# Aqasch/TensorRL-QAS

Hardware: AMD Instinct MI355X
Metric: VQE env-steps/sec (higher is better)
Workload: dtype f64

## Files before the change

### include/vqe_hip.h

```cpp
#ifndef VQE_HIP_H
#define VQE_HIP_H

#include <stdint.h>

#ifdef __cplusplus
extern "C" {
#endif

typedef struct vqe_handle vqe_t;
typedef struct vqe_cobyla vqe_cobyla_t;

enum {
  VQE_OK = 0,
  VQE_EINVAL = -22,
  VQE_ENOMEM = -12,
  VQE_ENODEV = -19,
  VQE_EHIP = -5,
  VQE_ESTATE = -1
};

enum {
  VQE_GATE_CNOT = 0,
  VQE_GATE_RX = 1,
  VQE_GATE_RY = 2,
  VQE_GATE_RZ = 3,
  VQE_GATE_DEPOL1 = 4,
  VQE_GATE_DEPOL2 = 5
};

int vqe_create(int n_qubits, int device_id, vqe_t** out);
void vqe_destroy(vqe_t* h);
const char* vqe_last_error(const vqe_t* h);
int vqe_set_stream(vqe_t* h, void* hip_stream);
int vqe_get_stream(vqe_t* h, void** hip_stream);
int vqe_sync(vqe_t* h);
int vqe_device_info(vqe_t* h, int64_t info[4]);

int vqe_set_init_state(vqe_t* h, const double* amps_re_im );
int vqe_set_init_state_dev(vqe_t* h, const void* dev_amps_re_im);
int vqe_get_state_dev(vqe_t* h, const double* theta, void* dev_amps_re_im);
int vqe_set_hamiltonian_pauli(vqe_t* h, int n_terms, const uint64_t* xmask,
                              const uint64_t* zmask, const double* coeff);
int vqe_set_hamiltonian_dense(vqe_t* h, const double* op_re_im , double tol);
int vqe_hamiltonian_terms(vqe_t* h, int32_t* n_terms, int32_t* n_xgroups);
int vqe_hamiltonian_layout(vqe_t* h, int32_t out[4]);
int vqe_set_term_shard(vqe_t* h, int rank, int world);
int vqe_set_amplitude_shard(vqe_t* h, int rank, int world);
int vqe_comm_unique_id(void* id128);
int vqe_comm_init(vqe_t* h, int rank, int world, const void* id128);
int vqe_comm_allreduce_energy(vqe_t* h);
int vqe_comm_destroy(vqe_t* h);
int vqe_term_owner(int n_qubits, int n_terms, const uint64_t* xmask, int world, int32_t* owner);
int vqe_set_noise(vqe_t* h, double p1, double p2, uint64_t seed);
int vqe_set_noise_mode(vqe_t* h, int mode);
int vqe_dm_plan(int n_qubits, int n_gates, const int32_t* kind, const int32_t* q0, const int32_t* q1, const int32_t* param_idx,
                const double* theta, double p1, double p2, int cap_blocks, int32_t* n_blocks, int32_t* windows, double* S);
int vqe_noise_mode_info(vqe_t* h, int32_t out[2]);
int vqe_set_shot_noise(vqe_t* h, double sigma_total, uint64_t seed);

int vqe_set_circuit(vqe_t* h, int n_gates, const int32_t* kind, const int32_t* q0,
                    const int32_t* q1, const int32_t* param_idx, int n_params);
int vqe_energy(vqe_t* h, const double* theta, double* energy);
int vqe_energy_batch(vqe_t* h, int batch, const double* theta ,
                     double* energy );
int vqe_energy_grad_batch(vqe_t* h, int batch, const double* theta ,
                          double* energy , double* grad );
int vqe_get_state(vqe_t* h, const double* theta, double* amps_re_im );
int vqe_minimize_cobyla(vqe_t* h, const double* x0, double rhobeg, double rhoend,
// ... 35 lines not shown
```

### tensorrl-qas_amd/_lib.py

```python
from __future__ import annotations

import ctypes as C
import os

try:
    import torch
except ImportError:
    torch = None

_HERE = os.path.dirname(os.path.abspath(__file__))
LIB_PATH = os.environ.get("VQE_HIP_LIB") or os.path.join(_HERE, "libvqe_hip.so")

c_i32p = C.POINTER(C.c_int32)
c_i64p = C.POINTER(C.c_int64)
c_u64p = C.POINTER(C.c_uint64)
c_f64p = C.POINTER(C.c_double)
vp = C.c_void_p

SIGNATURES = {
    "vqe_create": (C.c_int, [C.c_int, C.c_int, C.POINTER(vp)]),
    "vqe_destroy": (None, [vp]),
    "vqe_last_error": (C.c_char_p, [vp]),
    "vqe_set_stream": (C.c_int, [vp, vp]),
    "vqe_get_stream": (C.c_int, [vp, C.POINTER(vp)]),
    "vqe_sync": (C.c_int, [vp]),
    "vqe_device_info": (C.c_int, [vp, c_i64p]),
    "vqe_set_init_state": (C.c_int, [vp, c_f64p]),
    "vqe_set_hamiltonian_pauli": (C.c_int, [vp, C.c_int, c_u64p, c_u64p, c_f64p]),
    "vqe_set_hamiltonian_dense": (C.c_int, [vp, c_f64p, C.c_double]),
    "vqe_hamiltonian_terms": (C.c_int, [vp, c_i32p, c_i32p]),
    "vqe_hamiltonian_layout": (C.c_int, [vp, c_i32p]),
    "vqe_comm_unique_id": (C.c_int, [vp]),
    "vqe_comm_init": (C.c_int, [vp, C.c_int, C.c_int, vp]),
    "vqe_comm_allreduce_energy": (C.c_int, [vp]),
    "vqe_comm_destroy": (C.c_int, [vp]),
    "vqe_set_noise_mode": (C.c_int, [vp, C.c_int]),
    "vqe_noise_mode_info": (C.c_int, [vp, c_i32p]),
    "vqe_dm_plan": (C.c_int, [C.c_int, C.c_int, c_i32p, c_i32p, c_i32p, c_i32p, c_f64p, C.c_double, C.c_double, C.c_int, c_i32p,
                              c_i32p, c_f64p]),
    "vqe_set_init_state_dev": (C.c_int, [vp, vp]),
    "vqe_get_state_dev": (C.c_int, [vp, c_f64p, vp]),
    "vqe_set_term_shard": (C.c_int, [vp, C.c_int, C.c_int]),
    "vqe_set_amplitude_shard": (C.c_int, [vp, C.c_int, C.c_int]),
    "vqe_term_owner": (C.c_int, [C.c_int, C.c_int, c_u64p, C.c_int, c_i32p]),
    "vqe_set_noise": (C.c_int, [vp, C.c_double, C.c_double, C.c_uint64]),
    "vqe_set_shot_noise": (C.c_int, [vp, C.c_double, C.c_uint64]),
    "vqe_set_circuit": (C.c_int, [vp, C.c_int, c_i32p, c_i32p, c_i32p, c_i32p, C.c_int]),
    "vqe_energy": (C.c_int, [vp, c_f64p, c_f64p]),
    "vqe_energy_batch": (C.c_int, [vp, C.c_int, c_f64p, c_f64p]),
    "vqe_energy_grad_batch": (C.c_int, [vp, C.c_int, c_f64p, c_f64p, c_f64p]),
    "vqe_get_state": (C.c_int, [vp, c_f64p, c_f64p]),
    "vqe_minimize_cobyla": (C.c_int, [vp, c_f64p, C.c_double, C.c_double, C.c_int, c_f64p, c_f64p, c_i32p]),
    "vqe_batch_load": (C.c_int, [vp, C.c_int, c_i64p, c_i32p, c_i32p, c_i32p, c_i32p, c_i64p, c_f64p]),
    "vqe_batch_run_energy": (C.c_int, [vp]),
# ... 102 lines not shown
```

### tensorrl-qas_amd/csrc/vqe_api.hip

```cpp
#include "../../include/vqe_hip.h"
#include "vqe_device.h"
#include "vqe_stream.h"
#include "vqe_dm.h"
#include "vqe_grad.h"

#include <algorithm>
#include <cmath>
#include <complex>
#include <cstdio>
#include <cstdlib>
#include <cstring>
#include <dlfcn.h>
#include <map>
#include <new>
#include <string>
#include <vector>

using namespace vqe;

namespace {

std::string g_create_error;

template <class T>
// ... 16 lines not shown
struct vqe_handle {
  int n = 0, dev = 0;
  bool lds_path = true;
  int cu_count = 0, lds_per_cu = 0, last_wg_per_cu = 0;
  hipStream_t own_stream = nullptr, stream = nullptr;
  hipEvent_t ev0 = nullptr, ev1 = nullptr;
  float last_ms = 0.f;
  std::string err;

  DevBuf<double2> init;
  std::vector<uint32_t> gx_all;
  std::vector<std::vector<int>> group_terms;
  std::vector<uint64_t> hx, hz;
  std::vector<double> hcr, hci;
  int shard_rank = 0, shard_world = 1;
  int amp_rank = 0, amp_world = 1;
  bool ham_set = false;
  DevBuf<uint32_t> d_gx, d_term_z;
  DevBuf<double> d_term_cr, d_term_ci, d_tables;
  DevBuf<int32_t> d_tab_r, d_tab_i;

  DevBuf<int32_t> d_term_off;
  DevBuf<uint32_t> d_urec;
  DevBuf<double> d_utab;
  HamDev ham{};
  NoiseCfg noise{0.0, 0.0, 0ull, 0ull, 0.0};

  std::vector<GateRec> circ;
  int circ_params = -1;

  int batch = 0;
  int64_t total_params = 0;
  int max_ops = 0, max_params = 0, max_pair = 0;
  std::vector<int64_t> h_par_begin;
  std::vector<int32_t> h_par_count;
  DevBuf<GateRec> d_gates;
  DevBuf<int64_t> d_gate_begin, d_par_begin, d_scratch_begin;
  DevBuf<int32_t> d_gate_count, d_par_count, d_nfev, d_new_gate, d_order;
  bool has_new_gate = false;
  std::vector<int32_t> h_gate_count;
  std::vector<GateRec> h_gates;
  std::vector<int64_t> h_gate_begin;
  std::vector<double> h_theta;
  std::vector<int32_t> h_new_gate;
  DevBuf<GateRec> d_gates2;
  DevBuf<int64_t> d_gate_begin2, d_par_begin2;
  DevBuf<int32_t> d_gate_count2, d_par_count2;
  DevBuf<double> d_theta, d_x, d_xraw, d_f, d_scratch;
// ... 211 lines not shown
    uint32_t seen = 0;
    for (uint32_t p0 : act) {
      uint32_t key = 0;
      for (size_t i = 0; i < fixed.size(); ++i) key |= ((p0 >> fixed[i]) & 1u) << i;
      key |= ((p0 >> extra) & 1u) << fixed.size();
      seen |= 1u << key;
    }
    return __builtin_popcount(seen);
  };
  while ((int)fixed.size() < F) {
    int best = -1, best_cnt = 1 << 30;
    for (int b = n - 1; b >= 0; --b) {
      if (b == sel || std::find(fixed.begin(), fixed.end(), b) != fixed.end()) continue;
      const int c = count(b);
      if (c < best_cnt) { best_cnt = c; best = b; }
    }
    if (best < 0 || best_cnt >= 2 * patterns) break;
    fixed.push_back(best);
    patterns = best_cnt;
  }
  return patterns;
}

int build_hamiltonian(vqe_t* h) {
  const int n = h->n;
  ++h->gen;
  ++h->ham_ver;
  const std::vector<int> owner = assign_groups(h->gx_all, h->group_terms, h->lds_path, h->shard_world);
  std::vector<int> mine;
  for (size_t g = 0; g < owner.size(); ++g) if (owner[g] == h->shard_rank) mine.push_back((int)g);
  std::sort(mine.begin(), mine.end());

  std::vector<uint32_t> gx;
  std::vector<int32_t> term_off{0};
  std::vector<uint32_t> term_z;
  std::vector<double> term_cr, term_ci;
  const size_t dim = (size_t)1 << n;
  std::vector<int32_t> tab_r, tab_i;
  std::vector<double> tables;
  auto group_has_im = [&](int g) {
    for (int k : h->group_terms[g]) if (h->hci[k] != 0.0) return true;
    return false;
  };
  const bool reg_path = h->lds_path && n >= kRegMinQubits;
  const int lt = geo_lt(n);
  IndexMap im = identity_map(n), pm = identity_map(n);
  const int unit_F = n - 1 - lt;
  static const bool units_on = [] { const char* e = std::getenv("VQE_UNITS"); return !(e && e[0] == '0'); }();
  std::vector<char> sparse(h->gx_all.size(), 0);
  bool any_sparse = false;
  if (h->lds_path && n >= kUnitMinQubits && units_on && unit_F >= 1) {
    std::vector<int> hole_freq(n, 0);
    std::vector<uint32_t> dense_xs;
    std::vector<double> D;
    std::vector<uint32_t> act;
    std::vector<int> fixed;
    for (int g : mine) {
      const uint32_t x = h->gx_all[g];
      if (!x || group_has_im(g)) continue;
      const int sel = 31 - __builtin_clz(x);
      double scale;
      pair_table(h, g, im, n, sel, D, &scale);
      act.clear();
      for (size_t q = 0; q < D.size(); ++q)
        if (std::fabs(D[q]) > kUnitZeroTol * scale)
          act.push_back((uint32_t)(((q >> sel) << (sel + 1)) | (q & (((size_t)1 << sel) - 1))));
      const int patterns = choose_fixed_bits(n, sel, unit_F, act, fixed);
      const int units = patterns << (unit_F - (int)fixed.size());
      if (2 * units <= (1 << unit_F)) {
        sparse[g] = 1;
        any_sparse = true;
        for (int b : fixed) ++hole_freq[b];
        ++hole_freq[sel];
      } else {
        dense_xs.push_back(x);
      }
    }
    if (any_sparse && reg_path) {
      pm = choose_permutation(n, lt, dense_xs, hole_freq);
      im = pm;
      if (kUnitShear) {
        for (int i = 0; i < 4 && i < n; ++i)
          for (int j = 4; j < 8 && j < n; ++j)
            if ((kSwzCode[j - 4] >> i) & 1u) im.row[i] ^= pm.row[j];
        finish_inverse(im);
      }
    }
  }
  if (reg_path && !any_sparse) {
    std::vector<uint32_t> xs;
    for (int g : mine) if (h->gx_all[g] && !group_has_im(g)) xs.push_back(h->gx_all[g]);
    im = choose_index_map(n, lt, xs);
  }
  std::vector<uint32_t> urec;
  std::vector<double> utab;
  if (any_sparse) {
    const size_t NT = (size_t)1 << lt;
    std::vector<double> D;
    std::vector<uint32_t> act;
    std::vector<int> fixed;
    for (int g : mine) {
      if (!sparse[g]) continue;
      const uint32_t x = pm.map_x(h->gx_all[g]);
      const int sel = 31 - __builtin_clz(x);
      double scale;
      pair_table(h, g, pm, n, sel, D, &scale);
      auto rep = [&](size_t q) { return (uint32_t)(((q >> sel) << (sel + 1)) | (q & (((size_t)1 << sel) - 1))); };
      act.clear();
      for (size_t q = 0; q < D.size(); ++q) if (std::fabs(D[q]) > kUnitZeroTol * scale) act.push_back(rep(q));
      choose_fixed_bits(n, sel, unit_F, act, fixed);
      for (int b = n - 1; b >= 0 && (int)fixed.size() < unit_F; --b)
        if (b != sel && std::find(fixed.begin(), fixed.end(), b) == fixed.end()) fixed.push_back(b);
      uint32_t fmask = 0;
      for (int b : fixed) fmask |= 1u << b;
      uint32_t seen_keys[8];
      int n_keys = 0;
      for (uint32_t p0 : act) {
        const uint32_t key = p0 & fmask;
        bool dup = false;
        for (int i = 0; i < n_keys; ++i) dup |= seen_keys[i] == key;
        if (!dup && n_keys < 8) seen_keys[n_keys++] = key;
      }
      std::sort(seen_keys, seen_keys + n_keys);
      std::vector<int> holes(fixed);
      holes.push_back(sel);
      std::sort(holes.begin(), holes.end());
      uint32_t m[5] = {0, 0, 0, 0, 0};
      for (size_t i = 0; i <= holes.size(); ++i) {
        const int lo = i == 0 ? 0 : holes[i - 1] + 1, hi = i == holes.size() ? n : holes[i];
        m[i] = (uint32_t)((((uint64_t)1 << hi) - ((uint64_t)1 << lo)) << 4);
      }
      for (int ki = 0; ki < n_keys; ++ki) {
        const uint32_t s = seen_keys[ki];
        const uint32_t toff = (uint32_t)(utab.size() * sizeof(double));
        const uint32_t rec[8] = {m[0], m[1], m[2], m[3], m[4], (kUnitShear ? swz_index(s) : s) << 4, (kUnitShear ? swz_index(x) : x) << 4, toff};
        urec.insert(urec.end(), rec, rec + 8);
        for (size_t t = 0; t < NT; ++t) {
          uint32_t p0 = s, tb = 0;
          for (int b = 0; b < n; ++b)
            if (!((fmask >> b) & 1u) && b != sel) { p0 |= (uint32_t)((t >> tb) & 1u) << b; ++tb; }
          const size_t q = ((size_t)(p0 >> (sel + 1)) << sel) | (p0 & (((size_t)1 << sel) - 1));
          const double d = D[q];
          utab.push_back(std::fabs(d) > kUnitZeroTol * scale ? d : 0.0);
        }
      }
    }
    if (utab.size() * sizeof(double) + (size_t)kUnitUnroll * NT * sizeof(double) > 0x7FFFFFFFu)
      return fail(h, VQE_EINVAL, "Hamiltonian too large for the LDS-resident path");
    while ((urec.size() / 8) % kUnitUnroll) {
      const uint32_t rec[8] = {0, 0, 0, 0, 0, 0, 0, (uint32_t)(utab.size() * sizeof(double))};
      urec.insert(urec.end(), rec, rec + 8);
      utab.resize(utab.size() + NT, 0.0);
    }
    {
      std::vector<double> t(utab.size());
      const size_t n_trips = urec.size() / 8 / kUnitTrip;
      for (size_t T = 0; T < n_trips; ++T)
        for (size_t j = 0; j < (size_t)kUnitTrip; ++j)
          for (size_t th = 0; th < NT; ++th)
            t[(T * NT + th) * kUnitTrip + j] = utab[(T * kUnitTrip + j) * NT + th];
      utab.swap(t);
    }
  }
  auto gxm = [&](int g) { return im.map_x(h->gx_all[g]); };
  auto rank_of = [&](int g) {
    if (group_has_im(g)) return 3;
    const uint32_t x = gxm(g);
    if (x == 0) return 0;
    return reg_path && (x >> lt) ? 1 : 2;
  };
  auto top_bit = [&](int g) { const uint32_t x = gxm(g); return x ? 31 - __builtin_clz(x) : -1; };
  if (h->lds_path)
    std::stable_sort(mine.begin(), mine.end(), [&](int a, int b) {
      return rank_of(a) != rank_of(b) ? rank_of(a) < rank_of(b) : top_bit(a) > top_bit(b);
    });
  int has_diag = 0, n_real = 0, n_cls = 0;
  auto add_dummy = [&](uint32_t xd) {
    gx.push_back(xd);
    term_off.push_back((int32_t)term_z.size());
    tab_r.push_back((int32_t)tables.size());
    tab_i.push_back(-1);
    tables.resize(tables.size() + dim / 2, 0.0);
  };
  int cur_rank = 0;
  auto enter_section = [&](int rank) {
// ... 35 lines not shown
          const int cls = hb - lt;
          const uint32_t t = (uint32_t)((q >> 1) & (((size_t)1 << lt) - 1));
          const uint32_t j = (uint32_t)(((q >> (lt + 1)) << 1) | (q & 1));
          const uint32_t r = ((j >> cls) << (cls + 1)) | (j & ((1u << cls) - 1u));
          pidx[q] = t | (r << lt);
        } else {
          pidx[q] = (uint32_t)(((q >> hb) << (hb + 1)) | (q & (((size_t)1 << hb) - 1)));
        }
      }
      for (int k : h->group_terms[g]) {
        const uint32_t z = im.map_z((uint32_t)h->hz[k]);
        for (size_t q = 0; q < len; ++q) {
          const double sgn = ((__builtin_popcount(pidx[q] & z) & 1) ? -1.0 : 1.0) * (x == 0 ? 1.0 : 2.0);
          tr[q] += sgn * h->hcr[k];
          if (ti) ti[q] += sgn * h->hci[k];
        }
      }
    } else {
      tab_r.push_back(0);
      tab_i.push_back(has_im ? 0 : -1);
    }
  }
  enter_section(4);
  int rc;
  if ((rc = upload(h, h->d_gx, gx.data(), gx.size()))) return rc;
  if ((rc = upload(h, h->d_tab_r, tab_r.data(), tab_r.size()))) return rc;
  if ((rc = upload(h, h->d_tab_i, tab_i.data(), tab_i.size()))) return rc;
  if ((rc = upload(h, h->d_tables, tables.data(), tables.size()))) return rc;
  if ((rc = upload(h, h->d_term_off, term_off.data(), term_off.size()))) return rc;
  if ((rc = upload(h, h->d_term_z, term_z.data(), term_z.size()))) return rc;
  if ((rc = upload(h, h->d_term_cr, term_cr.data(), term_cr.size()))) return rc;
  if ((rc = upload(h, h->d_term_ci, term_ci.data(), term_ci.size()))) return rc;
  if ((rc = upload(h, h->d_urec, urec.data(), urec.size()))) return rc;
  if ((rc = upload(h, h->d_utab, utab.data(), utab.size()))) return rc;
  HIP_TRY(h, hipStreamSynchronize(h->stream));
  h->ham.n_groups = (int)gx.size();
  h->ham.n_terms = (int)term_z.size();
  h->ham.gx = h->d_gx.p;
  h->ham.tab_r = h->d_tab_r.p;
  h->ham.tab_i = h->d_tab_i.p;
  h->ham.tables = h->d_tables.p;
  h->ham.has_diag = has_diag;
  h->ham.n_real = n_real;
  h->ham.n_cls = n_cls;
  for (int i = 0; i < 16; ++i) h->ham.mrow[i] = im.row[i];
  h->ham.n_units = (int)(urec.size() / 8);
  h->ham.urec = h->d_urec.p;
  h->ham.utab = h->d_utab.p;
  h->ham.term_off = h->d_term_off.p;
  h->ham.term_z = h->d_term_z.p;
  h->ham.term_cr = h->d_term_cr.p;
  h->ham.term_ci = h->d_term_ci.p;
  return VQE_OK;
}

int check_gates(vqe_t* h, int64_t n_gates, const int32_t* kind, const int32_t* q0,
                const int32_t* q1, const int32_t* pidx, int n_params) {
  for (int64_t i = 0; i < n_gates; ++i) {
    const int k = kind[i];
    if (k < 0 || k > VQE_GATE_DEPOL2) return fail(h, VQE_EINVAL, "unknown gate kind");
    if (q0[i] < 0 || q0[i] >= h->n) return fail(h, VQE_EINVAL, "gate qubit out of range");
    if (k == VQE_GATE_CNOT || k == VQE_GATE_DEPOL2) {
      if (q1[i] < 0 || q1[i] >= h->n || q1[i] == q0[i])
        return fail(h, VQE_EINVAL, "two-qubit gate needs two distinct qubits in range");
    }
    if (k >= VQE_GATE_RX && k <= VQE_GATE_RZ) {
      if (pidx[i] < 0 || pidx[i] >= n_params)
        return fail(h, VQE_EINVAL, "rotation parameter index out of range");
    }
  }
// ... 990 lines not shown
  Rccl& r = rccl();
  const int rc = r.AllReduce(h->d_f.p, h->d_f.p, (size_t)h->batch,  8,  0, h->comm, h->stream);
  return rc ? fail(h, VQE_EHIP, std::string("ncclAllReduce: ") + (r.GetErrorString ? r.GetErrorString(rc) : "error")) : VQE_OK;
}

int vqe_comm_destroy(vqe_t* h) {
  if (!h) return VQE_EINVAL;
  if (h->comm) {
    (void)hipStreamSynchronize(h->stream);
    (void)rccl().CommDestroy(h->comm);
    h->comm = nullptr;
    h->comm_world = 0;
  }
  return VQE_OK;
}

int vqe_hamiltonian_layout(vqe_t* h, int32_t out[4]) {
  if (!h || !out) return VQE_EINVAL;
  if (!h->ham_set) return fail(h, VQE_ESTATE, "no Hamiltonian set");
  out[0] = h->ham.n_groups; out[1] = h->ham.n_units; out[2] = h->ham.n_cls; out[3] = h->ham.has_diag;
  return VQE_OK;
}

int vqe_set_term_shard(vqe_t* h, int rank, int world) {
  if (!h) return VQE_EINVAL;
  if (world < 1 || rank < 0 || rank >= world) return fail(h, VQE_EINVAL, "bad shard rank/world");
  h->shard_rank = rank;
  h->shard_world = world;
  if (h->ham_set) { HIP_TRY(h, hipSetDevice(h->dev)); return build_hamiltonian(h); }
  return VQE_OK;
}

int vqe_set_amplitude_shard(vqe_t* h, int rank, int world) {
  if (!h) return VQE_EINVAL;
  if (world < 1 || rank < 0 || rank >= world) return fail(h, VQE_EINVAL, "bad shard rank/world");
  if (h->lds_path && world > 1)
    return fail(h, VQE_ESTATE, "amplitude sharding of the energy sweep exists on the streaming path (n >= 14); use vqe_set_term_shard");
  const size_t blocks = ((size_t)1 << h->n) >> kETileBits;
  if (!h->lds_path && (blocks % (size_t)world) != 0) return fail(h, VQE_EINVAL, "world must divide the number of sweep tiles of the energy reduction");
  h->amp_rank = rank;
  h->amp_world = world;
  ++h->gen;
  return VQE_OK;
}

int vqe_set_noise(vqe_t* h, double p1, double p2, uint64_t seed) {
// ... 363 lines not shown
```

### tensorrl-qas_amd/csrc/vqe_device.h

```cpp
#pragma once
#include <hip/hip_runtime.h>
#include <stdint.h>
#ifdef VQE_STAMPS
__device__ unsigned long long g_cby_dbg[8];
__device__ unsigned long long g_cby_in_out[2];
__device__ long long g_cby_t0_unused;
#if defined(__HIP_DEVICE_COMPILE__)
#define CBY_STAMP_RESET() long long cby_t0_ = (long long)__builtin_readcyclecounter(); (void)cby_t0_
#define CBY_STAMP(k)                                                                               \
  {                                                                                                \
    const long long t_ = (long long)__builtin_readcyclecounter();                                  \
    if (ctx.tid == 0 && Ctx::nth > 1) __hip_atomic_fetch_add(&g_cby_dbg[k], (unsigned long long)(t_ - cby_t0_), __ATOMIC_RELAXED, __HIP_MEMORY_SCOPE_AGENT); \
    cby_t0_ = (long long)__builtin_readcyclecounter();                                             \
  }
#else
#define CBY_STAMP_RESET()
#define CBY_STAMP(k)
#endif
#endif
#include "cobyla_m0.h"

namespace vqe {

constexpr int kThreads = 256;
// ... 33 lines not shown

typedef int v4i_t __attribute__((ext_vector_type(4)));
typedef int v2i_t __attribute__((ext_vector_type(2)));
typedef double d2v_t __attribute__((ext_vector_type(2)));
typedef __attribute__((address_space(3))) const unsigned char lds_cbyte;
typedef __attribute__((address_space(3))) double lds_double;

enum : int { G_CNOT = 0, G_RX = 1, G_RY = 2, G_RZ = 3, G_DEPOL1 = 4, G_DEPOL2 = 5 };
enum : int { OP_RX = 1, OP_RY = 2, OP_RZ = 3, OP_PZ = 4, OP_NOP = 6 };

struct GateRec { int32_t kind, q0, q1, pidx; };
struct Op { uint32_t xm, zm; int32_t pidx; int32_t kind; };

struct HamDev {
  int n_groups;
  const uint32_t* gx;
  const int32_t* tab_r;
  const int32_t* tab_i;
  const double* tables;
  int has_diag;
  int n_real;
  int n_cls;
  uint32_t mrow[16];
  int n_units;
  const uint32_t* urec;
  const double* utab;
  int n_terms;
  const int32_t* term_off;
  const uint32_t* term_z;
  const double* term_cr;
  const double* term_ci;
};

constexpr uint32_t kSwzCode[4] = {1u, 15u, 2u, 12u};
constexpr unsigned long long kSwzTable = 0x1fe23dccd32ef10ull;
__host__ __device__ constexpr uint32_t swz_index(uint32_t p) {
  return p ^ (((p >> 4) & 1u) * kSwzCode[0]) ^ (((p >> 5) & 1u) * kSwzCode[1]) ^ (((p >> 6) & 1u) * kSwzCode[2]) ^
         (((p >> 7) & 1u) * kSwzCode[3]);
}
constexpr int kUnitMinQubits = 8;
constexpr int kUnitTrip = 4;
constexpr int kUnitUnroll = 3 * kUnitTrip;

struct NoiseCfg { double p1, p2; uint64_t seed; uint64_t eval_base; double shot_sigma; };

struct BatchArgs {
  int n;
  int batch;
  const GateRec* gates;
  const int64_t* gate_begin;
  const int32_t* gate_count;
  const int64_t* par_begin;
  const int32_t* par_count;
  const int32_t* order;
  const double* theta;
  double* xout;
  double* xraw;
  const int32_t* new_gate;
  int env_step;
  double* fout;
  int32_t* nfev;
// ... 329 lines not shown
  l.tile = cobyla_tile_bytes(n, max_params)
               ? (double*)((unsigned char*)l.psi + ((lds_bytes_base(n, max_ops, max_params, n_groups, max_pair) + 15) & ~(size_t)15) +
                           cobyla_resident_bytes(n, max_ops, max_params, n_groups, max_pair))
               : nullptr;
  return l;
}

__device__ __forceinline__ void stage_groups(const HamDev& H, const Lds& L) {
  for (int g = threadIdx.x; g < H.n_groups; g += (int)blockDim.x) {
    const uint32_t x = H.gx[g];
    L.gm[g] = GroupMeta{x, x ? 31 - __clz((int)x) : 0, H.tab_r[g], H.tab_i[g]};
  }
}

template <int N>
__device__ __forceinline__ void stage_cls(const HamDev& H, const Lds& L) {
  constexpr int LT = Geo<N>::LT;
  constexpr int NP = 1 << (N - LT - 1);
  for (int i = threadIdx.x; i < H.n_cls; i += (int)blockDim.x) {
    const uint32_t x = H.gx[i + H.has_diag];
    const int cls = (31 - __clz((int)x)) - LT;
    const uint32_t xr = x >> LT;
    uint32_t* w = (uint32_t*)(L.cm + i);
    w[0] = (x & ((1u << LT) - 1u)) << 4;
    w[1] = (uint32_t)cls;
    w[2] = w[3] = 0u;
    for (int j = 0; j < 8; ++j) w[4 + j] = j < NP ? ((insert0((uint32_t)j, cls) ^ xr) << (LT + 4)) : 0u;
  }
}

__device__ __forceinline__ void compile_ops(const BatchArgs& A, int b, uint64_t , const Lds& L, int skip = -1,
                                            bool slots = false, int skip_end = 0) {
  const int n = A.n;
  const int G = A.gate_count[b];
  const int cap = n >= 10 ? (ops_fit_upper_half(n, A.max_ops) ? (int)(((size_t)1 << n) / 2) : 0)
                          : (int)(((size_t)16 << n) / sizeof(GateRec));
  const GateRec* gsrc = A.gates + A.gate_begin[b];
  GateRec* gl = (GateRec*)L.psi;
  const bool staged = G <= cap;
  if (staged) {
    const int4* s4 = (const int4*)gsrc;
    int4* d4 = (int4*)gl;
    for (int i = threadIdx.x; i < G; i += (int)blockDim.x) d4[i] = s4[i];
  }
  __syncthreads();
  if (threadIdx.x == 0) {
    const GateRec* g = staged ? gl : gsrc;
// ... 512 lines not shown
        "v"(b[0].x), "v"(b[0].y), "v"(b[1].x), "v"(b[1].y), "v"(b[2].x), "v"(b[2].y), "v"(b[3].x), "v"(b[3].y),
        "v"(d0), "v"(d1), "v"(d2), "v"(d3));
}
__device__ __forceinline__ void pair_fma2(double& acc0, double& acc1, const double2& a0, const double2& a1,
                                          const double2 (&b)[2], double d0, double d1) {
  double t0, t1;
  asm("v_mul_f64 %2, %4, %8\n\tv_mul_f64 %3, %6, %10\n\t"
      "v_fmac_f64 %2, %5, %9\n\tv_fmac_f64 %3, %7, %11\n\t"
      "v_fmac_f64 %0, %2, %12\n\tv_fmac_f64 %1, %3, %13"
      : "+v"(acc0), "+v"(acc1), "=&v"(t0), "=&v"(t1)
      : "v"(a0.x), "v"(a0.y), "v"(a1.x), "v"(a1.y), "v"(b[0].x), "v"(b[0].y), "v"(b[1].x), "v"(b[1].y),
        "v"(d0), "v"(d1));
}
__device__ __forceinline__ void pair_fma1(double& acc0, const double2& a0, const double2 (&b)[1], double d0) {
  double t0;
  asm("v_mul_f64 %1, %2, %4\n\tv_fmac_f64 %1, %3, %5\n\tv_fmac_f64 %0, %1, %6"
      : "+v"(acc0), "=&v"(t0) : "v"(a0.x), "v"(a0.y), "v"(b[0].x), "v"(b[0].y), "v"(d0));
}

__device__ __forceinline__ double2 lds_load_abs(uint32_t addr) {
  const d2v_t v = *(const __attribute__((address_space(3))) d2v_t*)(uintptr_t)addr;
  return make_double2(v.x, v.y);
}
#ifndef VQE_UNIT_SHEAR
#define VQE_UNIT_SHEAR 0
#endif
constexpr bool kUnitShear = VQE_UNIT_SHEAR != 0;
typedef uint32_t u32x8_t __attribute__((ext_vector_type(8)));
typedef __attribute__((address_space(4))) const u32x8_t const_u32x8;

template <int N>
__device__ __forceinline__ void unit_energy(const Lds& L, const HamDev& H, double& acc0, double& acc1) {
  constexpr int LT = Geo<N>::LT;
  constexpr int SEG = (N - 1 - LT) + 2;
  static_assert(SEG >= 2 && SEG <= 5, "unit records hold five deposit masks");
  constexpr int U = kUnitTrip;
  static_assert(kUnitUnroll == 3 * kUnitTrip, "three trips per turn of the loop (ring of three table buffers)");
  constexpr uint32_t TSTRIDE = (uint32_t)8 << LT;
  static_assert(U == 4, "the tables of a trip are interleaved [thread][unit of the trip]: two 16-byte loads per thread and trip");
  constexpr uint32_t TRIP_BYTES = U * TSTRIDE;
  const int nu = __builtin_amdgcn_readfirstlane(H.n_units);
  if (nu <= 0) return;
  uint32_t tid = threadIdx.x;
  asm volatile("" : "+v"(tid));
  const __amdgpu_buffer_rsrc_t ru = table_rsrc(H.utab);
  const const_u32x8* rec = (const const_u32x8*)H.urec;
  uint32_t tsh[SEG];
#pragma unroll
  for (int i = 0; i < SEG; ++i) tsh[i] = tid << (4 + i);
  double d[3][U];
  u32x8_t R[U];
#pragma unroll
  for (int j = 0; j < U; ++j) {
    R[j] = rec[j];
  }
  const uint32_t tid32 = tid << 5;
  auto load_trip = [&](double (&dst)[U], uint32_t first_unit) {
    const uint32_t soff = (first_unit / U) * TRIP_BYTES;
    const double2 lo = buf_load_d2(ru, tid32, soff), hi = buf_load_d2(ru, tid32 + 16u, soff);
    dst[0] = lo.x; dst[1] = lo.y; dst[2] = hi.x; dst[3] = hi.y;
  };
  load_trip(d[0], 0u);
  load_trip(d[1], (uint32_t)(U < nu ? U : 0));
  const int last = nu - U;
  for (int u = 0; u < nu; u += 3 * U) {
#pragma unroll
    for (int k = 0; k < 3; ++k) {
      const int ub = u + k * U;
      const int u1 = ub + U < last ? ub + U : last;
      const int u2 = ub + 2 * U < last ? ub + 2 * U : last;
      double2 pa[U], pb[U];
      uint32_t a[U], ax[U];
#pragma unroll
      for (int j = 0; j < U; ++j) {
        uint32_t v;
        asm("v_and_b32 %0, %1, %2" : "=v"(v) : "s"(R[j][0]), "v"(tsh[0]));
#pragma unroll
        for (int i = 1; i < SEG; ++i) asm("v_and_or_b32 %0, %1, %2, %0" : "+v"(v) : "v"(tsh[i]), "s"(R[j][i]));
        if constexpr (kUnitShear) {
          const uint32_t u4 = (v >> 6) & 0x3Cu;
          v ^= ((uint32_t)(kSwzTable >> u4) << 4) & 0xF0u;
        }
        a[j] = v ^ R[j][5];
        ax[j] = a[j] ^ R[j][6];
      }
      __builtin_amdgcn_sched_barrier(0);
#pragma unroll
      for (int j = 0; j < U; ++j) {
        pb[j] = lds_load_abs(a[j]);
        pa[j] = lds_load_abs(ax[j]);
      }
      load_trip(d[(k + 2) % 3], (uint32_t)u2);
      __builtin_amdgcn_sched_barrier(0);
      const const_u32x8* rn = rec + u1;
#pragma unroll
      for (int j = 0; j < U; ++j) R[j] = rn[j];
      __builtin_amdgcn_sched_barrier(0);
#pragma unroll
      for (int j = 0; j < U; ++j) {
        const double v = (pa[j].x * pb[j].x + pa[j].y * pb[j].y) * d[k][j];
        if (j & 1) acc1 += v; else acc0 += v;
      }
      __builtin_amdgcn_sched_barrier(0);
    }
  }
}

struct NoHook { __device__ __forceinline__ void operator()() const {} };

template <int N, class Hook = NoHook>
__device__ __forceinline__ double reg_energy(const Lds& L, const HamDev& H, Hook after_pairs = Hook()) {
  constexpr int kThreads = Geo<N>::NT;
  constexpr uint32_t DIM = 1u << N;
  constexpr int LT = Geo<N>::LT;
  constexpr int R = N - LT;
  constexpr int NA = 1 << R;
  constexpr int NP = NA / 2;
  constexpr int HP = NP / 2;
  constexpr int PD = energy_pd(N);
  static_assert(NP >= 2 && NP <= 8 && PD % 2 == 0, "register energy path: 2..8 pairs per thread");
  uint32_t tid = threadIdx.x;
  asm volatile("" : "+v"(tid));
  const double* __restrict__ tables = H.tables;
  lds_cbyte* psi_l = (lds_cbyte*)L.psi;
  double2 own[NA];
#pragma unroll
  for (int r = 0; r < NA; ++r) own[r] = lds_load_d2(psi_l, (tid + (uint32_t)r * kThreads) << 4);
  double acc0 = 0.0, acc1 = 0.0;
  int g0 = 0;
  if (H.has_diag) {
    const __amdgpu_buffer_rsrc_t rd = table_rsrc(tables + __builtin_amdgcn_readfirstlane(L.gm[0].off_r));
#pragma unroll
    for (int r = 0; r < NA; ++r) {
      const double v = (own[r].x * own[r].x + own[r].y * own[r].y) * buf_load_d(rd, (tid + (uint32_t)r * kThreads) << 3, 0);
      if (r & 1) acc1 += v; else acc0 += v;
    }
    g0 = 1;
  }
  const int gc = g0 + H.n_cls;
  if (g0 < gc) {
    const int ncls = H.n_cls;
    constexpr uint32_t GSTRIDE = DIM * 4;
    double2 buf[PD][NP / 2];
    const __amdgpu_buffer_rsrc_t rt = table_rsrc(tables + __builtin_amdgcn_readfirstlane(L.gm[g0].off_r));
    uint32_t voff[NP / 2];
#pragma unroll
    for (int k = 0; k < NP / 2; ++k) voff[k] = (tid + (uint32_t)k * kThreads) << 4;
#pragma unroll
    for (int j = 0; j < PD - 1; ++j) {
#pragma unroll
      for (int k = 0; k < NP / 2; ++k) buf[j][k] = buf_load_d2(rt, voff[k], (uint32_t)j * GSTRIDE);
      __builtin_amdgcn_sched_barrier(0);
    }
#pragma unroll
    for (int k = 0; k < NP / 2; ++k) buf[PD - 1][k] = make_double2(0.0, 0.0);
    double2 bA[HP], bB[HP];
    uint2 mh[2];
    uint4 mo[2][2];
    const uint32_t tid16 = tid << 4;
    uint32_t tb;
    int ccls;
#define VQE_R_FETCH(S, GI)                                                                         \
    {                                                                                              \
      const ClsMeta* cm_ = L.cm + ((GI) < ncls ? (GI) : ncls - 1);                                 \
      mh[S] = *(const uint2*)cm_;                                                                  \
      mo[S][0] = *(const uint4*)cm_->off;                                                          \
      if constexpr (NP > 4) mo[S][1] = *(const uint4*)(cm_->off + 4);                             \
    }
#define VQE_R_OFF(S, J) ((J) == 0 ? mo[S][0].x : (J) == 1 ? mo[S][0].y : (J) == 2 ? mo[S][0].z : (J) == 3 ? mo[S][0].w : \
                         (J) == 4 ? mo[S][1].x : (J) == 5 ? mo[S][1].y : (J) == 6 ? mo[S][1].z : mo[S][1].w)
#define VQE_R_LOAD(S, HH, PB)                                                                      \
    _Pragma("unroll") for (int kk = 0; kk < HP; ++kk)                                             \
      PB[kk] = lds_load_d2(psi_l, tb + VQE_R_OFF(S, (HH) * HP + kk));
#define VQE_R_OWN(C, J) own[(((J) >> (C)) << ((C) + 1)) | ((J) & ((1 << (C)) - 1))]
#define VQE_R_DV(D, J) (((J) & 1) ? D[(J) / 2].y : D[(J) / 2].x)
#define VQE_R_COMP_C(C, HH, PB, D)                                                                 \
    if constexpr (HP == 4)                                                                         \
      pair_fma4(acc0, acc1, VQE_R_OWN(C, (HH) * 4), VQE_R_OWN(C, (HH) * 4 + 1), VQE_R_OWN(C, (HH) * 4 + 2),     \
                VQE_R_OWN(C, (HH) * 4 + 3), PB, VQE_R_DV(D, (HH) * 4), VQE_R_DV(D, (HH) * 4 + 1),            \
                VQE_R_DV(D, (HH) * 4 + 2), VQE_R_DV(D, (HH) * 4 + 3));                                       \
    else if constexpr (HP == 2)                                                                    \
      pair_fma2(acc0, acc1, VQE_R_OWN(C, (HH) * 2), VQE_R_OWN(C, (HH) * 2 + 1), PB, VQE_R_DV(D, (HH) * 2),     \
// ... 472 lines not shown
```

### tensorrl-qas_amd/engine.py

```python
from __future__ import annotations

import ctypes as C

import numpy as np

from . import _lib
from ._lib import VQEError, c_f64p, c_i32p, c_i64p, c_u64p

GATE_CNOT, GATE_RX, GATE_RY, GATE_RZ, GATE_DEPOL1, GATE_DEPOL2 = range(6)


def _f64(a):
    return np.ascontiguousarray(a, dtype=np.float64)


def _i32(a):
    return np.ascontiguousarray(a, dtype=np.int32)


def _i64(a):
    return np.ascontiguousarray(a, dtype=np.int64)


def _p(a, t):
# ... 84 lines not shown

    def set_hamiltonian(self, xmask, zmask, coeff):
        x = np.ascontiguousarray(xmask, dtype=np.uint64)
        z = np.ascontiguousarray(zmask, dtype=np.uint64)
        c = _f64(coeff)
        if not (x.size == z.size == c.size):
            raise ValueError("xmask, zmask, coeff differ in length")
        self._chk(self._lib.vqe_set_hamiltonian_pauli(self._h, int(x.size), _p(x, c_u64p), _p(z, c_u64p), _p(c, c_f64p)))

    def set_hamiltonian_dense(self, op, tol: float = 1e-13):
        a = np.ascontiguousarray(op, dtype=np.complex128)
        dim = 1 << self.n_qubits
        if a.shape != (dim, dim):
            raise ValueError("operator has the wrong shape")
        self._chk(self._lib.vqe_set_hamiltonian_dense(self._h, a.view(np.float64).ctypes.data_as(c_f64p), float(tol)))
        nt, ng = C.c_int32(), C.c_int32()
        self._chk(self._lib.vqe_hamiltonian_terms(self._h, C.byref(nt), C.byref(ng)))
        return nt.value, ng.value

    def hamiltonian_layout(self):
        out = (C.c_int32 * 4)()
        self._chk(self._lib.vqe_hamiltonian_layout(self._h, out))
        return {"table_groups": out[0], "units": out[1], "class_groups": out[2], "has_diag": bool(out[3])}

    @staticmethod
    def comm_unique_id() -> bytes:
        buf = C.create_string_buffer(128)
        rc = _lib.load().vqe_comm_unique_id(buf)
        if rc:
            raise VQEError(f"vqe_comm_unique_id failed ({rc})")
        return buf.raw

    def comm_init(self, rank: int, world: int, unique_id: bytes):
        buf = C.create_string_buffer(bytes(unique_id), 128)
        self._chk(self._lib.vqe_comm_init(self._h, int(rank), int(world), buf))

    def comm_allreduce_energy(self):
        self._chk(self._lib.vqe_comm_allreduce_energy(self._h))

    def comm_destroy(self):
        self._chk(self._lib.vqe_comm_destroy(self._h))

    def set_term_shard(self, rank: int, world: int):
        self._chk(self._lib.vqe_set_term_shard(self._h, int(rank), int(world)))

    def set_amplitude_shard(self, rank: int, world: int):
# ... 207 lines not shown
```

Before: 12380.

## Precompute unit LDS addresses and pick per-Hamiltonian bank swizzle by host search

Replaces the per-unit deposit-mask address computation in the sparse unit energy loop with precomputed per-thread LDS addresses loaded from a new device table, so unit records shrink to one xor mask. On the host it adds a greedy search over XOR swizzle codes that scores LDS bank conflicts for the actual unit addresses and applies the chosen swizzle to addresses, index-map rows and the register path's thread slots. This trades ALU work and the fixed compile-time shear for extra global memory traffic per trip and more host build time. It also exposes the bank-conflict scores through a new API call.

```diff
diff --git a/include/vqe_hip.h b/include/vqe_hip.h
--- a/include/vqe_hip.h
+++ b/include/vqe_hip.h
@@ -44,6 +44,7 @@
 int vqe_set_hamiltonian_dense(vqe_t* h, const double* op_re_im , double tol);
 int vqe_hamiltonian_terms(vqe_t* h, int32_t* n_terms, int32_t* n_xgroups);
 int vqe_hamiltonian_layout(vqe_t* h, int32_t out[4]);
+int vqe_unit_bank_score(vqe_t* h, double out[4]);
 int vqe_set_term_shard(vqe_t* h, int rank, int world);
 int vqe_set_amplitude_shard(vqe_t* h, int rank, int world);
 int vqe_comm_unique_id(void* id128);
diff --git a/tensorrl-qas_amd/_lib.py b/tensorrl-qas_amd/_lib.py
--- a/tensorrl-qas_amd/_lib.py
+++ b/tensorrl-qas_amd/_lib.py
@@ -30,6 +30,7 @@
     "vqe_set_hamiltonian_dense": (C.c_int, [vp, c_f64p, C.c_double]),
     "vqe_hamiltonian_terms": (C.c_int, [vp, c_i32p, c_i32p]),
     "vqe_hamiltonian_layout": (C.c_int, [vp, c_i32p]),
+    "vqe_unit_bank_score": (C.c_int, [vp, c_f64p]),
     "vqe_comm_unique_id": (C.c_int, [vp]),
     "vqe_comm_init": (C.c_int, [vp, C.c_int, C.c_int, vp]),
     "vqe_comm_allreduce_energy": (C.c_int, [vp]),
diff --git a/tensorrl-qas_amd/csrc/vqe_api.hip b/tensorrl-qas_amd/csrc/vqe_api.hip
--- a/tensorrl-qas_amd/csrc/vqe_api.hip
+++ b/tensorrl-qas_amd/csrc/vqe_api.hip
@@ -62,8 +62,10 @@
 
   DevBuf<int32_t> d_term_off;
   DevBuf<uint32_t> d_urec;
+  DevBuf<uint32_t> d_uaddr;
   DevBuf<double> d_utab;
   HamDev ham{};
+  double unit_score[4] = {1.0, 1.0, 1.0, 1.0};
   NoiseCfg noise{0.0, 0.0, 0ull, 0ull, 0.0};
 
   std::vector<GateRec> circ;
@@ -321,6 +323,76 @@
   return patterns;
 }
 
+struct SwzChoice { uint64_t swz; double mean0, worst0, mean, worst; };
+SwzChoice choose_bank_swizzle(int lt, const std::vector<uint32_t>& urec, const std::vector<uint32_t>& addr) {
+  const size_t NT = (size_t)1 << lt, nu = urec.size();
+  std::vector<uint8_t> lo, hi;
+  size_t n_scored = 0;
+  for (size_t u = 0; u < nu; ++u) {
+    if (!urec[u]) continue;
+    ++n_scored;
+    for (size_t t = 0; t < NT; ++t) {
+      const uint32_t p = addr[((u / kUnitTrip) * NT + t) * kUnitTrip + u % kUnitTrip] >> 4;
+      lo.push_back((uint8_t)(p & 15u));
+      hi.push_back((uint8_t)((p >> 4) & 15u));
+    }
+  }
+  uint8_t grp[4][16];
+  for (int g = 0, cnt[4] = {0, 0, 0, 0}; g < 64; ++g) {
+    const int k = ((g >> 5) << 1) | (((g >> 2) ^ (g >> 3) ^ (g >> 4)) & 1);
+    grp[k][cnt[k]++] = (uint8_t)g;
+  }
+  auto table = [](const uint32_t (&c)[4]) {
+    uint64_t t = 0;
+    for (uint32_t v = 0; v < 16; ++v) {
+      uint32_t code = 0;
+      for (int k = 0; k < 4; ++k) if ((v >> k) & 1u) code ^= c[k];
+      t |= (uint64_t)code << (4 * v);
+    }
+    return t;
+  };
+  auto score = [&](uint64_t swz, double* worst) {
+    size_t tot = 0;
+    int w = 1;
+    for (size_t i = 0; i < n_scored * NT; i += 64)
+      for (int k = 0; k < 4; ++k) {
+        int seen[16] = {0}, m = 0;
+        for (int l = 0; l < 16; ++l) {
+          const size_t j = i + grp[k][l];
+          const int s = lo[j] ^ (int)((swz >> (4 * hi[j])) & 15u);
+          m = std::max(m, ++seen[s]);
+        }
+        tot += m;
+        w = std::max(w, m);
+      }
+    if (worst) *worst = w;
+    return n_scored ? (double)tot / (double)(n_scored * NT / 16) : 1.0;
+  };
+  SwzChoice r{0, 1.0, 1.0, 1.0, 1.0};
+  if (!n_scored || lt < 8) return r;
+  r.mean0 = r.mean = score(0, &r.worst0);
+  r.worst = r.worst0;
+  const uint32_t starts[2][4] = {{0u, 0u, 0u, 0u}, {1u, 15u, 2u, 12u}};
+  for (const auto& st : starts) {
+    uint32_t c[4] = {st[0], st[1], st[2], st[3]};
+    double best = score(table(c), nullptr);
+    for (int sweep = 0; sweep < 4; ++sweep) {
+      bool moved = false;
+      for (int k = 0; k < 4; ++k)
+        for (uint32_t v = 0; v < 16; ++v) {
+          const uint32_t keep = c[k];
+          c[k] = v;
+          const double s = score(table(c), nullptr);
+          if (s < best) { best = s; moved = true; } else c[k] = keep;
+        }
+      if (!moved) break;
+    }
+    if (best < r.mean) { r.mean = best; r.swz = table(c); }
+  }
+  if (r.swz) score(r.swz, &r.worst);
+  return r;
+}
+
 int build_hamiltonian(vqe_t* h) {
   const int n = h->n;
   ++h->gen;
@@ -343,7 +415,7 @@
   };
   const bool reg_path = h->lds_path && n >= kRegMinQubits;
   const int lt = geo_lt(n);
-  IndexMap im = identity_map(n), pm = identity_map(n);
+  IndexMap im = identity_map(n);
   const int unit_F = n - 1 - lt;
   static const bool units_on = [] { const char* e = std::getenv("VQE_UNITS"); return !(e && e[0] == '0'); }();
   std::vector<char> sparse(h->gx_all.size(), 0);
@@ -375,23 +447,15 @@
         dense_xs.push_back(x);
       }
     }
-    if (any_sparse && reg_path) {
-      pm = choose_permutation(n, lt, dense_xs, hole_freq);
-      im = pm;
-      if (kUnitShear) {
-        for (int i = 0; i < 4 && i < n; ++i)
-          for (int j = 4; j < 8 && j < n; ++j)
-            if ((kSwzCode[j - 4] >> i) & 1u) im.row[i] ^= pm.row[j];
-        finish_inverse(im);
-      }
-    }
+    if (any_sparse && reg_path)
+      im = choose_permutation(n, lt, dense_xs, hole_freq);
   }
   if (reg_path && !any_sparse) {
     std::vector<uint32_t> xs;
     for (int g : mine) if (h->gx_all[g] && !group_has_im(g)) xs.push_back(h->gx_all[g]);
     im = choose_index_map(n, lt, xs);
   }
-  std::vector<uint32_t> urec;
+  std::vector<uint32_t> urec, uaddr;
   std::vector<double> utab;
   if (any_sparse) {
     const size_t NT = (size_t)1 << lt;
@@ -400,10 +464,10 @@
     std::vector<int> fixed;
     for (int g : mine) {
       if (!sparse[g]) continue;
-      const uint32_t x = pm.map_x(h->gx_all[g]);
+      const uint32_t x = im.map_x(h->gx_all[g]);
       const int sel = 31 - __builtin_clz(x);
       double scale;
-      pair_table(h, g, pm, n, sel, D, &scale);
+      pair_table(h, g, im, n, sel, D, &scale);
       auto rep = [&](size_t q) { return (uint32_t)(((q >> sel) << (sel + 1)) | (q & (((size_t)1 << sel) - 1))); };
       act.clear();
       for (size_t q = 0; q < D.size(); ++q) if (std::fabs(D[q]) > kUnitZeroTol * scale) act.push_back(rep(q));
@@ -421,19 +485,9 @@
         if (!dup && n_keys < 8) seen_keys[n_keys++] = key;
       }
       std::sort(seen_keys, seen_keys + n_keys);
-      std::vector<int> holes(fixed);
-      holes.push_back(sel);
-      std::sort(holes.begin(), holes.end());
-      uint32_t m[5] = {0, 0, 0, 0, 0};
-      for (size_t i = 0; i <= holes.size(); ++i) {
-        const int lo = i == 0 ? 0 : holes[i - 1] + 1, hi = i == holes.size() ? n : holes[i];
-        m[i] = (uint32_t)((((uint64_t)1 << hi) - ((uint64_t)1 << lo)) << 4);
-      }
       for (int ki = 0; ki < n_keys; ++ki) {
         const uint32_t s = seen_keys[ki];
-        const uint32_t toff = (uint32_t)(utab.size() * sizeof(double));
-        const uint32_t rec[8] = {m[0], m[1], m[2], m[3], m[4], (kUnitShear ? swz_index(s) : s) << 4, (kUnitShear ? swz_index(x) : x) << 4, toff};
-        urec.insert(urec.end(), rec, rec + 8);
+        urec.push_back(x << 4);
         for (size_t t = 0; t < NT; ++t) {
           uint32_t p0 = s, tb = 0;
           for (int b = 0; b < n; ++b)
@@ -441,25 +495,28 @@
           const size_t q = ((size_t)(p0 >> (sel + 1)) << sel) | (p0 & (((size_t)1 << sel) - 1));
           const double d = D[q];
           utab.push_back(std::fabs(d) > kUnitZeroTol * scale ? d : 0.0);
+          uaddr.push_back(p0 << 4);
         }
       }
     }
     if (utab.size() * sizeof(double) + (size_t)kUnitUnroll * NT * sizeof(double) > 0x7FFFFFFFu)
       return fail(h, VQE_EINVAL, "Hamiltonian too large for the LDS-resident path");
-    while ((urec.size() / 8) % kUnitUnroll) {
-      const uint32_t rec[8] = {0, 0, 0, 0, 0, 0, 0, (uint32_t)(utab.size() * sizeof(double))};
-      urec.insert(urec.end(), rec, rec + 8);
+    while (urec.size() % kUnitUnroll) {
+      urec.push_back(0u);
       utab.resize(utab.size() + NT, 0.0);
-    }
-    {
-      std::vector<double> t(utab.size());
-      const size_t n_trips = urec.size() / 8 / kUnitTrip;
+      uaddr.resize(uaddr.size() + NT, 0u);
+    }
+    auto by_trip = [&](auto& v) {
+      std::remove_reference_t<decltype(v)> t(v.size());
+      const size_t n_trips = urec.size() / kUnitTrip;
       for (size_t T = 0; T < n_trips; ++T)
         for (size_t j = 0; j < (size_t)kUnitTrip; ++j)
           for (size_t th = 0; th < NT; ++th)
-            t[(T * NT + th) * kUnitTrip + j] = utab[(T * kUnitTrip + j) * NT + th];
-      utab.swap(t);
-    }
+            t[(T * NT + th) * kUnitTrip + j] = v[(T * kUnitTrip + j) * NT + th];
+      v.swap(t);
+    };
+    by_trip(utab);
+    by_trip(uaddr);
   }
   auto gxm = [&](int g) { return im.map_x(h->gx_all[g]); };
   auto rank_of = [&](int g) {
@@ -541,6 +598,12 @@
     }
   }
   enter_section(4);
+  SwzChoice sw{0, 1.0, 1.0, 1.0, 1.0};
+  if (reg_path && !urec.empty() && gx.size() == (size_t)(has_diag + n_cls)) sw = choose_bank_swizzle(lt, urec, uaddr);
+  if (sw.swz) {
+    for (uint32_t& a : uaddr) a = swz_slot(sw.swz, a >> 4) << 4;
+    for (uint32_t& x : urec) x = swz_slot(sw.swz, x >> 4) << 4;
+  }
   int rc;
   if ((rc = upload(h, h->d_gx, gx.data(), gx.size()))) return rc;
   if ((rc = upload(h, h->d_tab_r, tab_r.data(), tab_r.size()))) return rc;
@@ -551,6 +614,7 @@
   if ((rc = upload(h, h->d_term_cr, term_cr.data(), term_cr.size()))) return rc;
   if ((rc = upload(h, h->d_term_ci, term_ci.data(), term_ci.size()))) return rc;
   if ((rc = upload(h, h->d_urec, urec.data(), urec.size()))) return rc;
+  if ((rc = upload(h, h->d_uaddr, uaddr.data(), uaddr.size()))) return rc;
   if ((rc = upload(h, h->d_utab, utab.data(), utab.size()))) return rc;
   HIP_TRY(h, hipStreamSynchronize(h->stream));
   h->ham.n_groups = (int)gx.size();
@@ -562,9 +626,17 @@
   h->ham.has_diag = has_diag;
   h->ham.n_real = n_real;
   h->ham.n_cls = n_cls;
-  for (int i = 0; i < 16; ++i) h->ham.mrow[i] = im.row[i];
-  h->ham.n_units = (int)(urec.size() / 8);
+  for (int i = 0; i < 16; ++i) {
+    uint32_t row = im.row[i];
+    for (int k = 0; i < 4 && k < 4; ++k)
+      if ((sw.swz >> (4 * (1 << k)) >> i) & 1u) row ^= im.row[4 + k];
+    h->ham.mrow[i] = row;
+  }
+  h->ham.swz = sw.swz;
+  h->unit_score[0] = sw.mean0; h->unit_score[1] = sw.worst0; h->unit_score[2] = sw.mean; h->unit_score[3] = sw.worst;
+  h->ham.n_units = (int)urec.size();
   h->ham.urec = h->d_urec.p;
+  h->ham.uaddr = h->d_uaddr.p;
   h->ham.utab = h->d_utab.p;
   h->ham.term_off = h->d_term_off.p;
   h->ham.term_z = h->d_term_z.p;
@@ -1601,6 +1673,13 @@
   return VQE_OK;
 }
 
+int vqe_unit_bank_score(vqe_t* h, double out[4]) {
+  if (!h || !out) return VQE_EINVAL;
+  if (!h->ham_set) return fail(h, VQE_ESTATE, "no Hamiltonian set");
+  for (int i = 0; i < 4; ++i) out[i] = h->unit_score[i];
+  return VQE_OK;
+}
+
 int vqe_set_term_shard(vqe_t* h, int rank, int world) {
   if (!h) return VQE_EINVAL;
   if (world < 1 || rank < 0 || rank >= world) return fail(h, VQE_EINVAL, "bad shard rank/world");
diff --git a/tensorrl-qas_amd/csrc/vqe_device.h b/tensorrl-qas_amd/csrc/vqe_device.h
--- a/tensorrl-qas_amd/csrc/vqe_device.h
+++ b/tensorrl-qas_amd/csrc/vqe_device.h
@@ -79,8 +79,10 @@
   int n_real;
   int n_cls;
   uint32_t mrow[16];
+  uint64_t swz;
   int n_units;
   const uint32_t* urec;
+  const uint32_t* uaddr;
   const double* utab;
   int n_terms;
   const int32_t* term_off;
@@ -89,11 +91,8 @@
   const double* term_ci;
 };
 
-constexpr uint32_t kSwzCode[4] = {1u, 15u, 2u, 12u};
-constexpr unsigned long long kSwzTable = 0x1fe23dccd32ef10ull;
-__host__ __device__ constexpr uint32_t swz_index(uint32_t p) {
-  return p ^ (((p >> 4) & 1u) * kSwzCode[0]) ^ (((p >> 5) & 1u) * kSwzCode[1]) ^ (((p >> 6) & 1u) * kSwzCode[2]) ^
-         (((p >> 7) & 1u) * kSwzCode[3]);
+__host__ __device__ inline uint32_t swz_slot(uint64_t swz, uint32_t p) {
+  return p ^ (uint32_t)((swz >> (((p >> 4) & 15u) << 2)) & 15u);
 }
 constexpr int kUnitMinQubits = 8;
 constexpr int kUnitTrip = 4;
@@ -469,7 +468,7 @@
     const int cls = (31 - __clz((int)x)) - LT;
     const uint32_t xr = x >> LT;
     uint32_t* w = (uint32_t*)(L.cm + i);
-    w[0] = (x & ((1u << LT) - 1u)) << 4;
+    w[0] = swz_slot(H.swz, x & ((1u << LT) - 1u)) << 4;
     w[1] = (uint32_t)cls;
     w[2] = w[3] = 0u;
     for (int j = 0; j < 8; ++j) w[4 + j] = j < NP ? ((insert0((uint32_t)j, cls) ^ xr) << (LT + 4)) : 0u;
@@ -1028,46 +1027,39 @@
   const d2v_t v = *(const __attribute__((address_space(3))) d2v_t*)(uintptr_t)addr;
   return make_double2(v.x, v.y);
 }
-#ifndef VQE_UNIT_SHEAR
-#define VQE_UNIT_SHEAR 0
-#endif
-constexpr bool kUnitShear = VQE_UNIT_SHEAR != 0;
-typedef uint32_t u32x8_t __attribute__((ext_vector_type(8)));
-typedef __attribute__((address_space(4))) const u32x8_t const_u32x8;
+typedef uint32_t u32x4_t __attribute__((ext_vector_type(4)));
+typedef __attribute__((address_space(4))) const u32x4_t const_u32x4;
 
 template <int N>
 __device__ __forceinline__ void unit_energy(const Lds& L, const HamDev& H, double& acc0, double& acc1) {
   constexpr int LT = Geo<N>::LT;
-  constexpr int SEG = (N - 1 - LT) + 2;
-  static_assert(SEG >= 2 && SEG <= 5, "unit records hold five deposit masks");
   constexpr int U = kUnitTrip;
   static_assert(kUnitUnroll == 3 * kUnitTrip, "three trips per turn of the loop (ring of three table buffers)");
-  constexpr uint32_t TSTRIDE = (uint32_t)8 << LT;
-  static_assert(U == 4, "the tables of a trip are interleaved [thread][unit of the trip]: two 16-byte loads per thread and trip");
-  constexpr uint32_t TRIP_BYTES = U * TSTRIDE;
+  static_assert(U == 4, "a trip is [thread][unit of the trip]: two 16-byte table loads and one 16-byte address load per thread");
+  constexpr uint32_t TRIP_BYTES = (uint32_t)(8 * U) << LT;
+  constexpr uint32_t TRIP_ABYTES = (uint32_t)(4 * U) << LT;
   const int nu = __builtin_amdgcn_readfirstlane(H.n_units);
   if (nu <= 0) return;
   uint32_t tid = threadIdx.x;
   asm volatile("" : "+v"(tid));
   const __amdgpu_buffer_rsrc_t ru = table_rsrc(H.utab);
-  const const_u32x8* rec = (const const_u32x8*)H.urec;
-  uint32_t tsh[SEG];
-#pragma unroll
-  for (int i = 0; i < SEG; ++i) tsh[i] = tid << (4 + i);
+  const __amdgpu_buffer_rsrc_t ra = table_rsrc(H.uaddr);
+  const const_u32x4* rec = (const const_u32x4*)H.urec;
   double d[3][U];
-  u32x8_t R[U];
-#pragma unroll
-  for (int j = 0; j < U; ++j) {
-    R[j] = rec[j];
-  }
+  u32x4_t ad[3];
+  u32x4_t X = rec[0];
   const uint32_t tid32 = tid << 5;
-  auto load_trip = [&](double (&dst)[U], uint32_t first_unit) {
-    const uint32_t soff = (first_unit / U) * TRIP_BYTES;
+  const uint32_t tid16 = tid << 4;
+  auto load_trip = [&](double (&dst)[U], u32x4_t& adst, uint32_t first_unit) {
+    const uint32_t trip = first_unit / U;
+    const v4i_t av = __builtin_amdgcn_raw_buffer_load_b128(ra, (int)tid16, (int)(trip * TRIP_ABYTES), 0);
+    adst = u32x4_t{(uint32_t)av.x, (uint32_t)av.y, (uint32_t)av.z, (uint32_t)av.w};
+    const uint32_t soff = trip * TRIP_BYTES;
     const double2 lo = buf_load_d2(ru, tid32, soff), hi = buf_load_d2(ru, tid32 + 16u, soff);
     dst[0] = lo.x; dst[1] = lo.y; dst[2] = hi.x; dst[3] = hi.y;
   };
-  load_trip(d[0], 0u);
-  load_trip(d[1], (uint32_t)(U < nu ? U : 0));
+  load_trip(d[0], ad[0], 0u);
+  load_trip(d[1], ad[1], (uint32_t)(U < nu ? U : 0));
   const int last = nu - U;
   for (int u = 0; u < nu; u += 3 * U) {
 #pragma unroll
@@ -1079,16 +1071,8 @@
       uint32_t a[U], ax[U];
 #pragma unroll
       for (int j = 0; j < U; ++j) {
-        uint32_t v;
-        asm("v_and_b32 %0, %1, %2" : "=v"(v) : "s"(R[j][0]), "v"(tsh[0]));
-#pragma unroll
-        for (int i = 1; i < SEG; ++i) asm("v_and_or_b32 %0, %1, %2, %0" : "+v"(v) : "v"(tsh[i]), "s"(R[j][i]));
-        if constexpr (kUnitShear) {
-          const uint32_t u4 = (v >> 6) & 0x3Cu;
-          v ^= ((uint32_t)(kSwzTable >> u4) << 4) & 0xF0u;
-        }
-        a[j] = v ^ R[j][5];
-        ax[j] = a[j] ^ R[j][6];
+        a[j] = ad[k][j];
+        asm("v_xor_b32 %0, %1, %2" : "=v"(ax[j]) : "s"(X[j]), "v"(a[j]));
       }
       __builtin_amdgcn_sched_barrier(0);
 #pragma unroll
@@ -1096,11 +1080,9 @@
         pb[j] = lds_load_abs(a[j]);
         pa[j] = lds_load_abs(ax[j]);
       }
-      load_trip(d[(k + 2) % 3], (uint32_t)u2);
+      load_trip(d[(k + 2) % 3], ad[(k + 2) % 3], (uint32_t)u2);
       __builtin_amdgcn_sched_barrier(0);
-      const const_u32x8* rn = rec + u1;
-#pragma unroll
-      for (int j = 0; j < U; ++j) R[j] = rn[j];
+      X = rec[u1 / U];
       __builtin_amdgcn_sched_barrier(0);
 #pragma unroll
       for (int j = 0; j < U; ++j) {
@@ -1127,11 +1109,12 @@
   static_assert(NP >= 2 && NP <= 8 && PD % 2 == 0, "register energy path: 2..8 pairs per thread");
   uint32_t tid = threadIdx.x;
   asm volatile("" : "+v"(tid));
+  const uint32_t stid = swz_slot(H.swz, tid);
   const double* __restrict__ tables = H.tables;
   lds_cbyte* psi_l = (lds_cbyte*)L.psi;
   double2 own[NA];
 #pragma unroll
-  for (int r = 0; r < NA; ++r) own[r] = lds_load_d2(psi_l, (tid + (uint32_t)r * kThreads) << 4);
+  for (int r = 0; r < NA; ++r) own[r] = lds_load_d2(psi_l, (stid + (uint32_t)r * kThreads) << 4);
   double acc0 = 0.0, acc1 = 0.0;
   int g0 = 0;
   if (H.has_diag) {
@@ -1163,7 +1146,7 @@
     double2 bA[HP], bB[HP];
     uint2 mh[2];
     uint4 mo[2][2];
-    const uint32_t tid16 = tid << 4;
+    const uint32_t tid16 = stid << 4;
     uint32_t tb;
     int ccls;
 #define VQE_R_FETCH(S, GI)                                                                         \
diff --git a/tensorrl-qas_amd/engine.py b/tensorrl-qas_amd/engine.py
--- a/tensorrl-qas_amd/engine.py
+++ b/tensorrl-qas_amd/engine.py
@@ -130,6 +130,11 @@
         out = (C.c_int32 * 4)()
         self._chk(self._lib.vqe_hamiltonian_layout(self._h, out))
         return {"table_groups": out[0], "units": out[1], "class_groups": out[2], "has_diag": bool(out[3])}
+
+    def unit_bank_score(self):
+        out = (C.c_double * 4)()
+        self._chk(self._lib.vqe_unit_bank_score(self._h, out))
+        return {"plain_mean": out[0], "plain_worst": out[1], "mean": out[2], "worst": out[3]}
 
     @staticmethod
     def comm_unique_id() -> bytes:
```

Result: faster. 13380 (median of 6 runs) (+8.1%).
